# tudoroancea/ihm2

Hardware: AMD Instinct MI355X
Metric: NMPC RTI solves/s (batch), N=40, nx=8 (6-DOF bicycle), fkin6 (higher is better)
Workload: dtype f64

## Files before the change

ihm2_amd/csrc/kernels_qp.hip:

```cpp
#include <cstring>

#include "ihm2mpc_internal.h"
#include "device_steps.hpp"
#include "sqp_body.hpp"
#include "irk_body.hpp"
#include "riccati_mfma.hpp"
#include "sens_body.hpp"
#include "qp_lds.hpp"
#include "qp_catalogue.hpp"
#include "wave_sync.hpp"

using namespace ihm2;

namespace {

#define INF_BOUND 1e20
#ifndef RIC_RING
#define RIC_RING 4
#endif
#ifndef SWEEP_RING
#define SWEEP_RING 4
#endif
#define SWEEP_DL ((SWEEP_RING >= 8) ? 4 : 2)

__device__ __forceinline__ bool fin(double v) { return fabs(v) < INF_BOUND; }
__device__ __forceinline__ int here(int v) { asm volatile("" : "+v"(v)); return v; }

template <typename OP>
__device__ __forceinline__ double wave_reduce(double v, OP op)
{
    v = op(v, dpp_mov<0xB1>(v));
    v = op(v, dpp_mov<0x4E>(v));
    v = op(v, dpp_mov<0x141>(v));
    v = op(v, dpp_mov<0x128>(v));
    int lo = __double2loint(v), hi = __double2hiint(v);
    auto a16 = __builtin_amdgcn_permlane16_swap(lo, lo, false, false);
    auto b16 = __builtin_amdgcn_permlane16_swap(hi, hi, false, false);
    v = op(__hiloint2double(b16[0], a16[0]), __hiloint2double(b16[1], a16[1]));
    lo = __double2loint(v); hi = __double2hiint(v);
    auto a32 = __builtin_amdgcn_permlane32_swap(lo, lo, false, false);
    auto b32 = __builtin_amdgcn_permlane32_swap(hi, hi, false, false);
    return op(__hiloint2double(b32[0], a32[0]), __hiloint2double(b32[1], a32[1]));
}
__device__ __forceinline__ double nanmax(double a, double b) { return (a != a || b != b) ? NAN : fmax(a, b); }
__device__ __forceinline__ double wave_max(double v) { return wave_reduce(v, [](double a, double b) { return fmax(a, b); }); }
__device__ __forceinline__ double wave_min(double v) { return wave_reduce(v, [](double a, double b) { return fmin(a, b); }); }
__device__ __forceinline__ double wave_sum(double v) { return wave_reduce(v, [](double a, double b) { return a + b; }); }
__device__ __forceinline__ double wave_nanmax(double v) { return wave_reduce(v, [](double a, double b) { return nanmax(a, b); }); }

__device__ __forceinline__ double sum8(double v)
{
    v += dpp_mov<0xB1>(v);
    v += dpp_mov<0x4E>(v);
    v += dpp_mov<0x141>(v);
    return v;
}

__device__ __forceinline__ double sum_stride8(double v)
{
    v += dpp_mov<0x128>(v);
    int lo = __double2loint(v), hi = __double2hiint(v);
    auto a16 = __builtin_amdgcn_permlane16_swap(lo, lo, false, false);
    auto b16 = __builtin_amdgcn_permlane16_swap(hi, hi, false, false);
    v = __hiloint2double(b16[0], a16[0]) + __hiloint2double(b16[1], a16[1]);
    lo = __double2loint(v); hi = __double2hiint(v);
    auto a32 = __builtin_amdgcn_permlane32_swap(lo, lo, false, false);
    auto b32 = __builtin_amdgcn_permlane32_swap(hi, hi, false, false);
    return __hiloint2double(b32[0], a32[0]) + __hiloint2double(b32[1], a32[1]);
}

template <int DIR, int D, int DL, bool BUF = true, typename P, typename F>
__device__ __forceinline__ void stream_rows(const double *rows, int N, int e_even, int e_odd, P &&pre, F &&body)
{
    static_assert(D % 2 == 0 && DL % 2 == 0 && D % DL == 0 && 3 * D <= QM_PAD, "the element index alternates with the step parity");
    double r[2][D], x0[DL], x1[DL];
    const __amdgpu_buffer_rsrc_t rsrc = __builtin_amdgcn_make_buffer_rsrc(const_cast<double *>(rows) - (size_t)QM_PAD * 64, 0, (N + 2 * QM_PAD) * 512, 0x00020000);
    const unsigned ve = (unsigned)e_even * 8u, vo = (unsigned)e_odd * 8u;
    typedef unsigned int u2_t __attribute__((ext_vector_type(2)));
    const double *p_even = rows + (size_t)((DIR < 0) ? N - 1 : 0) * 64 + e_even, *p_odd = rows + (size_t)((DIR < 0) ? N - 1 : 0) * 64 + e_odd;
    auto load_row = [&](const int step, const bool odd) -> double {
        if constexpr (BUF) {
            const int row = (DIR < 0) ? N - 1 - step : step;
            const u2_t v = __builtin_amdgcn_raw_buffer_load_b64(rsrc, odd ? vo : ve, (QM_PAD + row) * 512, 0);
            return __hiloint2double((int)v.y, (int)v.x);
        } else
            return (odd ? p_odd : p_even)[(ptrdiff_t)DIR * step * 64];
    };
#pragma unroll
    for (int d = 0; d < D; d++) {
        r[0][d] = load_row(d, (d & 1) != 0);
        __builtin_amdgcn_sched_barrier(0);
        if (d < DL) pre((DIR < 0) ? N - 1 - d : d, (d & 1) != 0, x0[d], x1[d]);
    }
    for (int s0 = 0; s0 < N; s0 += 2 * D) {
#pragma unroll
        for (int h = 0; h < 2; h++) {
#pragma unroll
            for (int d = 0; d < D; d++) {
                const int s = s0 + h * D + d;
                const int k = (DIR < 0) ? N - 1 - s : s;
                const double v = r[h][d], y0 = x0[d % DL], y1 = x1[d % DL];
                r[h ^ 1][d] = load_row(s + D, (d & 1) != 0);
                pre((DIR < 0) ? k - DL : k + DL, (d & 1) != 0, x0[d % DL], x1[d % DL]);
                if (s < N) body(k, v, (d & 1) != 0, y0, y1);
            }
        }
    }
}
template <int DIR, int D, int DL, typename P, typename F>
__device__ __forceinline__ void stream_rows_v1(const double *rows, int N, int e_even, int e_odd, P &&pre, F &&body)
{
    stream_rows<DIR, D, DL, false>(rows, N, e_even, e_odd, pre, body);
}

template <int NSLOT, int NSOFT, int PATH, int UNI, int NW = 1, int LEAN = 1, int NF = 0, int FULL = 0>
__device__ __forceinline__ void qp_wave_body(const QpArgs &a, const int b, double *sm, const bool want_res = true)
{
    static_assert(NF == 0 || NW == 1, "the straight-line factor sweep parks its idle lanes' stores in the tile the block reductions use");
    static_assert(FULL == 0 || (NSOFT == 0 && PATH == 0 && UNI != 0 && NW == 1 && LEAN != 0 && NF > 0 && NSLOT <= 8),
                  "the full slot form is written for the all-hard table of the batch-shared rows, one wave, the lean phases and the compiled-in horizon");
    constexpr int NT = 64 * NW;
    const int tid = threadIdx.x, lane = tid & 63, wv = tid >> 6;
#define BSYNC() do { if (NW == 1) WSYNC(); else __syncthreads(); } while (0)
    const int N = (NF > 0) ? NF : a.N, NS = N + 1;
    constexpr QpLdsClass CLS = qp_lds_class(PATH, UNI != 0);
    constexpr int NCK = CLS.nck;
    const double *Hs0 = a.Hs + (size_t)b * a.hs_bs, *HsT = Hs0 + a.hs_te;
    const double *Gy0 = a.Gy + (size_t)b * a.gy_bs, *GyT = Gy0 + a.gy_te;
    const double *slot_lbb = a.slot_lb + (size_t)b * a.sl_bs, *slot_ubb = a.slot_ub + (size_t)b * a.sl_bs;
    constexpr bool ALAT = PATH == 2;
    constexpr bool HL = CLS.hl, CL = CLS.cl;
    static_assert(qp_factor_inside(qp_lds(40, CLS), 40, NCK) && qp_factor_inside(qp_lds(2, CLS), 2, NCK), "factor stage / block reductions leave their LDS");
    static_assert(qp_sweeps_inside(qp_lds(40, CLS), 40, LEAN != 0, SWEEP_RING, SWEEP_DL) && (LEAN == 0 || qp_sweeps_inside(qp_lds(2, CLS), 2, true, SWEEP_RING, SWEEP_DL)),
                  "the sweeps' unclamped LDS prefetch leaves the block (the earlier form does below N = 4: api.hip refuses those launches)");
    static_assert(NW <= 4, "qp_factor_inside checks the block reductions for four waves");
    static_assert(FULL == 0 || qp_full_zeroes_kept(qp_lds(NF > 0 ? NF : 2, CLS), NF > 0 ? NF : 2), "a store of the factor sweep reaches gam or cf: the full slot form zeroes them once per solve");
#define LEN(id) qp_lds_len(id, N, NS, CLS)
    double *z = sm, *gt = z + LEN(QP_Z), *pi = gt + LEN(QP_GT), *pv = pi + LEN(QP_PI), *rb = pv + LEN(QP_PV), *gam = rb + LEN(QP_RB), *cf = gam + LEN(QP_GAM), *dz = cf + LEN(QP_CF);
    double *kff = dz + LEN(QP_DZ), *Kl = kff + LEN(QP_KFF), *Ginv = Kl + LEN(QP_KL), *Prb = Ginv + LEN(QP_GINV), *tile = Prb + LEN(QP_PRB), *hc = tile + LEN(QP_TILE), *ha = hc + LEN(QP_HC);
    double *Hl = ha + LEN(QP_HA), *CDl = Hl + LEN(QP_HL), *spv = CDl + LEN(QP_CDL);
    int *spc = reinterpret_cast<int *>(spv + 60);
#undef LEN
#define HS(k, i, l) (HL ? Hl[(((k) == N) ? 100 : 0) + (i) * 10 + (l)] : ((k) == N ? HsT : Hs0 + (UNI ? 0 : (k)) * 100)[(i) * 10 + (l)])
#define CDV(k, r, j) (CL ? CDl[(r) * 10 + (j)] : a.CD[((k) * 2 + (r)) * 10 + (j)])

    auto blk_reduce = [&](double v, auto op) -> double {
        v = wave_reduce(v, op);
        if (NW > 1) {
            __syncthreads();
            if (lane == 0) tile[wv] = v;
            __syncthreads();
            v = tile[0];
#pragma unroll
            for (int w = 1; w < NW; w++) v = op(v, tile[w]);
        }
        return v;
    };
    auto blk_max = [&](double v) { return blk_reduce(v, [](double x, double y) { return fmax(x, y); }); };
    auto blk_min = [&](double v) { return blk_reduce(v, [](double x, double y) { return fmin(x, y); }); };
    auto blk_sum = [&](double v) { return blk_reduce(v, [](double x, double y) { return x + y; }); };
    auto blk_nanmax = [&](double v) { return blk_reduce(v, [](double x, double y) { return nanmax(x, y); }); };

    const double *xb = a.x + (size_t)b * NS * 8;
    const double *ub = a.u + (size_t)b * N * 2;
    const double *linb = a.lin + (size_t)b * N * LIN_REC;
    double *gb = a.g + (size_t)b * NS * 10;
    double *rgb = a.rg + (size_t)b * NS * 10;
    double *Pg = a.P + (size_t)b * NS * 64;
    double *Mg = a.M + (size_t)b * N * 64;
    double *pib = a.pi + (size_t)b * NS * 8;
    double *lamb = a.lam + (size_t)b * NS * 28;
    double *slkb = a.slk + (size_t)b * NS * 28;
    double *lamab = ALAT ? a.lam_a + (size_t)b * NS * 2 : nullptr;
    double *slkab = ALAT ? a.slk_a + (size_t)b * NS * 2 : nullptr;
    auto alat_slot = [](int j) -> int { return (j == 3) ? 0 : (j == 4) ? 1 : (j == 6) ? 2 : (j == 7) ? 3 : -1; };

    if (HL) for (int e = tid; e < 200; e += NT) Hl[e] = (e < 100) ? Hs0[e] : HsT[e - 100];
    if (CL && tid < 20) CDl[tid] = a.CD[tid];
    if (UNI) BSYNC();
    bool h_sparse = false;
    if (HL) {
        int cnt = 0;
        if (tid < 20) {
#pragma unroll
            for (int l = 0; l < 10; l++) {
                const double v = Hl[tid * 10 + l];
                if (v != 0.0) { if (cnt < 3) { spv[tid * 3 + cnt] = v; spc[tid * 3 + cnt] = l; } cnt++; }
            }
            for (int q = cnt; q < 3; q++) { spv[tid * 3 + q] = 0.0; spc[tid * 3 + q] = 0; }
        }
        h_sparse = __ballot(cnt > 3) == 0ull;
        if (NW > 1) h_sparse = blk_max((wv == 0 && !h_sparse) ? 1.0 : 0.0) == 0.0;
        BSYNC();
    }
    double sg = 1.0, sb = 1.0, r_stat = 0.0, r_eq = 0.0;
    double w_R = 0.0, w_L = 0.0;
    if (PATH) {
        const int trk = a.track_id[b];
        w_R = a.widths[trk * 2 + 0]; w_L = a.widths[trk * 2 + 1];
        for (int k = tid; k < NS; k += NT) {
            const double psi = xb[k * 8 + 2], sgn = (psi > 0.0) - (psi < 0.0);
            const double dfoot = -0.5 * a.car_L * cos(fabs(psi)) * sgn, dlat = -0.5 * a.car_W * sin(psi);
            hc[k * 2 + 0] = (k >= 1) ? dfoot + dlat : 0.0;
            hc[k * 2 + 1] = (k >= 1) ? -dfoot + dlat : 0.0;
            if (ALAT) {
                double g4[4];
                alat_eval(xb[k * 8 + 3], xb[k * 8 + 4], xb[k * 8 + 6], xb[k * 8 + 7], g4);
#pragma unroll
                for (int q = 0; q < 4; q++) ha[k * 4 + q] = (k >= 1 && k < N) ? g4[q] : 0.0;
            }
        }
        BSYNC();
    }
    for (int e = tid; e < NS * 10; e += NT) {
        const int k = e / 10, j = e % 10;
        double acc = 0.0;
#pragma unroll
        for (int l = 0; l < 8; l++) acc = fma(HS(k, j, l), xb[k * 8 + l], acc);
        if (k < N) {
            acc = fma(HS(k, j, 8), ub[k * 2 + 0], acc);
            acc = fma(HS(k, j, 9), ub[k * 2 + 1], acc);
            const double *yr = a.yref + ((size_t)b * N + k) * 12;
#pragma unroll
            for (int l = 0; l < 12; l++) acc = fma(-Gy0[((UNI ? 0 : k) * 10 + j) * 12 + l], yr[l], acc);
        } else {
            const double *yr = a.yref_e + (size_t)b * 8;
#pragma unroll
            for (int l = 0; l < 8; l++) acc = fma(-GyT[j * 12 + l], yr[l], acc);
        }
        gb[e] = acc;
        const bool counted = !((k == 0 && j < 8) || (k == N && j >= 8));
        if (j < 8 || k < N) sg = fmax(sg, fabs(acc));
        if (!want_res) continue;
        double st = acc;
        if (k < N) {
            const double *rec = linb + (size_t)k * LIN_REC;
#pragma unroll
            for (int l = 0; l < 8; l++) st = fma((j < 8) ? rec[l * 8 + j] : rec[64 + l * 2 + (j - 8)], pib[(k + 1) * 8 + l], st);
        }
        if (j < 8) st -= pib[k * 8 + j];
        st -= lamb[k * 28 + j] - lamb[k * 28 + 14 + j];
        if (k < N) {
            st = fma(-CDV(k, 0, j), lamb[k * 28 + 10] - lamb[k * 28 + 24], st);
            st = fma(-CDV(k, 1, j), lamb[k * 28 + 11] - lamb[k * 28 + 25], st);
        }
        if (PATH && (j == 1 || j == 2)) {
            const double l12 = lamb[k * 28 + 12] - lamb[k * 28 + 26], l13 = lamb[k * 28 + 13] - lamb[k * 28 + 27];
            st -= (j == 1) ? l12 - l13 : hc[k * 2] * l12 + hc[k * 2 + 1] * l13;
        }
        if (ALAT && alat_slot(j) >= 0) st -= ha[k * 4 + alat_slot(j)] * (lamab[k * 2] - lamab[k * 2 + 1]);
        if (counted) r_stat = fmax(r_stat, fabs(st));
    }
    for (int e = tid; e < N * 8; e += NT) {
        const double bl = linb[(size_t)(e / 8) * LIN_REC + 80 + (e % 8)];
        sb = fmax(sb, fabs(bl));
        r_eq = fmax(r_eq, fabs(bl));
    }
    if (tid < 8) {
        const double d = a.x0[(size_t)b * 8 + tid] - xb[tid];
        sb = fmax(sb, fabs(d));
        r_eq = fmax(r_eq, fabs(d));
    }
    sg = blk_max(sg); sb = blk_max(sb);

    int s_kc[NSLOT];
    double s_dl[NSLOT], s_du[NSLOT];
    double lam_l[NSLOT], lam_u[NSLOT], t_l[NSLOT], t_u[NSLOT];
    constexpr int NSO = (NSOFT > 0) ? NSOFT : 1;
    double so_zw[NSO], so_Zw[NSO], so_s[NSO], so_ls[NSO], so_rs[NSO], so_ds[NSO], so_dls[NSO], so_pa[NSO];
#pragma unroll
    for (int r = 0; r < NSO; r++) { so_zw[r] = 0.0; so_Zw[r] = -1.0; so_s[r] = 1.0; so_ls[r] = 0.0; so_rs[r] = 0.0; so_ds[r] = so_dls[r] = so_pa[r] = 0.0; }
#define IS_SOFT(r) ((r) < NSOFT && so_Zw[(r) < NSOFT ? (r) : 0] >= 0.0)
#define ONE_SIDED(r) (NSOFT > 0 && PATH != 2 && (r) < NSOFT)
#define HAS_L(r) (FULL ? true : ONE_SIDED(r) ? true : fin(s_dl[r]))
// ... 158 lines not shown
            }
            __syncthreads();
            mu_acc = 0.0;
            for (int sidx = lane; sidx < a.nslots_can; sidx += 64) mu_acc = __dadd_rn(mu_acc, gam[sidx]);
            __syncthreads();
        }
        if (LEAN == 0) BSYNC();
        for (int rpass = 0; rpass < 2; rpass++) {
            if (exact) {
                for (int e = tid; e < NS * 10; e += NT) {
                    const int k = e / 10, j = e % 10;
                    double acc = gb[e];
                    if (HL && h_sparse) {
                        const int row = ((k == N) ? 10 : 0) + j;
#pragma unroll
                        for (int q = 0; q < 3; q++) acc = fma(spv[row * 3 + q], z[k * 10 + spc[row * 3 + q]], acc);
                    } else {
#pragma unroll
                        for (int l = 0; l < 10; l++) acc = fma(HS(k, j, l), z[k * 10 + l], acc);
                    }
                    if (k < N) {
                        acc = fma(-CDV(k, 0, j), cf[k * NCK + 10], acc);
                        acc = fma(-CDV(k, 1, j), cf[k * NCK + 11], acc);
                    }
                    if (j < 8) acc -= pi[k * 8 + j];
                    acc -= cf[k * NCK + j];
                    if (PATH && (j == 1 || j == 2)) {
                        const double l12 = cf[k * NCK + 12], l13 = cf[k * NCK + 13];
                        acc -= (j == 1) ? l12 - l13 : hc[k * 2] * l12 + hc[k * 2 + 1] * l13;
                    }
                    if (ALAT && alat_slot(j) >= 0) acc -= ha[k * 4 + alat_slot(j)] * cf[k * NCK + 14];
                    gt[e] = acc;
                }
                BSYNC();
                dyn_residual<4, NT>(N, tid, const_cast<double *>(linb), z, pi, gt, rb, LIN_REC);
                BSYNC();
            }
            res_g = 0.0; res_b = 0.0;
            if (exact || LEAN == 0) {
                for (int e = tid; e < NS * 10; e += NT) {
                    const int k = e / 10, j = e % 10;
                    double v = gt[e];
                    if ((k == 0 && j < 8) || (k == N && j >= 8)) { v = 0.0; gt[e] = 0.0; }
                    if (exact) rgb[e] = v;
                    res_g = nanmax(res_g, fabs(v));
                }
                for (int e = tid; e < N * 8; e += NT) res_b = nanmax(res_b, fabs(rb[e]));
            } else { res_g = fol_g; res_b = fol_b; }
            res_g = nanmax(res_g, res_gs);
            res_g = blk_nanmax(res_g); res_b = blk_nanmax(res_b);
            if (rpass == 0) { res_d = blk_nanmax(res_d); res_m = blk_nanmax(res_m); mu = ((NW == 1) ? blk_sum(mu_acc) : wave_sum(mu_acc)) * inv_m; }
            if (!(res_g == res_g) || !(res_b == res_b) || !(res_d == res_d) || !(res_m == res_m)) { qstatus = (it == 0) ? 3 : 4; finished = true; break; }
            const bool conv = res_g <= tol_g && res_b <= tol_b && res_d <= tol_d && res_m <= tol_m;
            if (conv && exact) { qstatus = 0; finished = true; break; }
            if ((conv || it >= a.iter_max) && !exact) {
                exact = true; exact_mode = true;
                if (LEAN != 0) multipliers_to_cf();
                continue;
            }
            break;
        }
        if (finished) break;
        if (it >= a.iter_max) { qstatus = 1; break; }
        BSYNC();
        double alpha = 1.0, alpha_d = 1.0, sigma = 0.0;
        auto slot_coeffs = [&](int pass) {
            if (!FULL) {
                for (int e = tid; e < NS * NCK; e += NT) { cf[e] = 0.0; if (pass == 0) gam[e] = 0.0; }
                BSYNC();
            }
            const double mu_t = fmax(sigma * mu, mu_floor);
#pragma unroll
            for (int r = 0; r < NSLOT; r++) {
                if (NO_SLOT(r)) continue;
                const bool al = HAS_L(r), au = HAS_U(r);
                double c = 0.0;
                if (IS_SOFT(r)) {
                    const int q = r < NSOFT ? r : 0;
                    const double lm = al ? lam_l[r] : lam_u[r], tt = al ? t_l[r] : t_u[r], rdv = al ? rd_l[r] : rd_u[r];
                    const double gm = lm / tt, gs = so_ls[q] / so_s[q], D = so_Zw[q] + gm + gs;
                    double c1, c2, rsv;
                    if (pass == 0) { c1 = (lm * tt + lm * rdv) / tt; c2 = so_ls[q]; rsv = so_rs[q]; SLOT_AT(gam, r) += gm * (so_Zw[q] + gs) / D; }
                    else { c1 = ((al ? pa_l[r] : pa_u[r]) - mu_t) / tt; c2 = (so_pa[q] - mu_t) / so_s[q]; rsv = 0.0; }
                    c = c1 - gm * (rsv + c1 + c2) / D;
                    SLOT_AT(cf, r) += ONE_SIDED(r) ? ROW_SIGN(r, c) : (al ? c : -c);
                    continue;
                }
                if (pass == 0) {
                    const double gl = al ? lam_l[r] / t_l[r] : 0.0, gu = au ? lam_u[r] / t_u[r] : 0.0;
                    if (al) c += fma(gl, rd_l[r], lam_l[r]);
                    if (au) c -= fma(gu, rd_u[r], lam_u[r]);
                    SLOT_ACC(SLOT_AT(gam, r), gl + gu);
                } else {
                    if (al) c += (pa_l[r] - mu_t) / t_l[r];
                    if (au) c -= (pa_u[r] - mu_t) / t_u[r];
                }
                SLOT_ACC(SLOT_AT(cf, r), ROW_SIGN(r, c));
            }
            BSYNC();
        };
        auto add_coeffs = [&]() {
            for (int e = tid; e < NS * 10; e += NT) {
                const int k = e / 10, j = e % 10;
                double acc = gt[e] + cf[k * NCK + j];
                if (k < N) {
                    acc = fma(CDV(k, 0, j), cf[k * NCK + 10], acc);
                    acc = fma(CDV(k, 1, j), cf[k * NCK + 11], acc);
                }
                if (PATH && (j == 1 || j == 2)) {
                    const double c12 = cf[k * NCK + 12], c13 = cf[k * NCK + 13];
                    acc += (j == 1) ? c12 - c13 : hc[k * 2] * c12 + hc[k * 2 + 1] * c13;
                }
                if (ALAT && alat_slot(j) >= 0) acc += ha[k * 4 + alat_slot(j)] * cf[k * NCK + 14];
                gt[e] = acc;
            }
            BSYNC();

        };
        slot_coeffs(0);
        add_coeffs();
        __builtin_amdgcn_s_waitcnt(0x0F70);
        if (wv == 0) {
            RicLds L;
            const QpRic o = qp_lds_ric(N, NS, NCK);
            L.gt = o.gt; L.pv = o.pv; L.gam = o.gam; L.dz = o.dz; L.kff = o.kff; L.Kl = o.Kl;
            L.Ginv = o.Ginv; L.hv = o.Prb; L.tile = o.tile; L.hc = o.hc; L.ha = o.ha;
            if constexpr (NF != 0)
                riccati_sweep_mfma<NCK, PATH != 0, UNI != 0, RIC_RING, ALAT, true, (NF > 0) ? NF : 0>(N, lane, linb, Hs0, HsT, a.CD, L, Pg, Mg, LIN_REC, false, false);
            else
            riccati_sweep_mfma<NCK, PATH != 0, UNI != 0, RIC_RING, ALAT>(N, lane, linb, Hs0, HsT, a.CD, L, Pg, Mg, LIN_REC, a.m_act == 0, a.symmetrize != 0);
            if (lane < 8) dz[lane] = 0.0;
        }
        BSYNC();
        for (int pass = 0; pass < 2; pass++) {
            const double mu_t = fmax(sigma * mu, mu_floor);
            if (pass == 1) slot_coeffs(1);
            if (pass == 1) {
            add_coeffs();
            for (int e = tid; e < NS * 8; e += NT) {
                const int k = e >> 3, j = e & 7;
                double v = gt[k * 10 + j];
                if (k < N) v -= Kl[k * 16 + j] * gt[k * 10 + 8] + Kl[k * 16 + 8 + j] * gt[k * 10 + 9];
                pv[e] = v;
            }
            BSYNC();
            if constexpr (LEAN != 0) {
            if (wv == 0) {
                const int g = lane >> 3, w = lane & 7;
                double pw = pv[N * 8 + w], pg = 0.0;
                const int se2 = (w == 0) ? 16 : 0, so2 = (g == 0) ? 16 : 0;
                const double *be = (w == 0) ? pv + (N - 1) * 8 + g : dz, *bo = (g == 0) ? pv + (N - 2) * 8 + w : dz;
                const double *qe = Prb + (N - 1) * 8 + w, *qo = Prb + (N - 2) * 8 + g;
                double *oe = pv + (N - 1) * 8 + g, *oo = pv + (N - 2) * 8 + w;
                stream_rows<-1, SWEEP_RING, SWEEP_DL>(Mg, N, RIC_IDX(w, g), RIC_IDX(g, w),
                    [&](int k, bool odd, double &prb, double &base) {
                        if (odd) { prb = *qo; qo -= 16; base = *bo; bo -= so2; } else { prb = *qe; qe -= 16; base = *be; be -= se2; }
                    },
                    [&](int k, double m, bool odd, double prb, double base) {
                        if (!odd) {
                            pg = sum8(fma(m, pw, fma(m, prb, base)));
                            *oe = pg; oe -= 16;
                        } else {
                            pw = sum_stride8(fma(m, pg, fma(m, prb, base)));
                            *oo = pw; oo -= 16;
                        }
                    });
            }
            } else {
            if (wv == 0) {
                const int g = lane >> 3, w = lane & 7;
                double pw = pv[N * 8 + w], pg = 0.0;
                stream_rows_v1<-1, QP_V1_RING, QP_V1_DL>(Mg, N, RIC_IDX(w, g), RIC_IDX(g, w),
                    [&](int k, bool odd, double &prb, double &base) { prb = Prb[k * 8 + (odd ? g : w)]; base = pv[k * 8 + (odd ? w : g)]; },
                    [&](int k, double m, bool odd, double prb, double base) {
                        if (!odd) {
                            const double off = fma(m, prb, (w == 0) ? base : 0.0);
                            pg = sum8(fma(m, pw, off));
                            if (w == 0) pv[k * 8 + g] = pg;
                        } else {
                            const double off = fma(m, prb, (g == 0) ? base : 0.0);
                            pw = sum_stride8(fma(m, pg, off));
                            if (g == 0) pv[k * 8 + w] = pw;
                        }
                    });
            }
            }
            BSYNC();
            for (int k = tid; k < N; k += NT) {
                const double *rec = linb + (size_t)k * LIN_REC;
                double g0 = gt[k * 10 + 8], g1 = gt[k * 10 + 9];
                double Bk[16];
#pragma unroll
                for (int l = 0; l < 16; l++) Bk[l] = rec[64 + l];
#pragma unroll
                for (int l = 0; l < 8; l++) {
                    const double h = Prb[k * 8 + l] + pv[(k + 1) * 8 + l];
                    g0 = fma(Bk[l * 2 + 0], h, g0);
                    g1 = fma(Bk[l * 2 + 1], h, g1);
                }
                const double kf0 = Ginv[k * 8 + 0] * g0 + Ginv[k * 8 + 1] * g1;
                const double kf1 = Ginv[k * 8 + 1] * g0 + Ginv[k * 8 + 2] * g1;
                kff[k * 4 + 0] = kf0;
                kff[k * 4 + 1] = kf1;
#pragma unroll
                for (int i = 0; i < 8; i++) dz[(k + 1) * 10 + i] = rb[k * 8 + i] - Bk[i * 2] * kf0 - Bk[i * 2 + 1] * kf1;
            }
            if (tid < 8) dz[tid] = 0.0;
            BSYNC();
            }

            if constexpr (LEAN != 0) {
            if (wv == 0) {
                const int g = lane >> 3, w = lane & 7;
                double dxw = dz[w], dxg = 0.0;
                const int se2 = (w == 0) ? 20 : 0, so2 = (g == 0) ? 20 : 0;
                const double *ce = (w == 0) ? dz + 10 + g : dz, *co = (g == 0) ? dz + 20 + w : dz;
                stream_rows<+1, SWEEP_RING, SWEEP_DL>(Mg, N, RIC_IDX(g, w), RIC_IDX(w, g),
                    [&](int k, bool odd, double &c, double &unused) {
                        if (odd) { c = *co; co += so2; } else { c = *ce; ce += se2; }
                        unused = 0.0;
                    },
                    [&](int k, double m, bool odd, double c, double) {
                        if (!odd) {
                            dxg = sum8(fma(m, dxw, c));
                            dz[(k + 1) * 10 + g] = dxg;
                        } else {
                            dxw = sum_stride8(fma(m, dxg, c));
                            dz[(k + 1) * 10 + w] = dxw;
                        }
                    });
            }
            } else {
            if (wv == 0) {
                const int g = lane >> 3, w = lane & 7;
                double dxw = dz[w], dxg = 0.0;
                stream_rows_v1<+1, QP_V1_RING, QP_V1_DL>(Mg, N, RIC_IDX(g, w), RIC_IDX(w, g),
                    [&](int k, bool odd, double &c, double &unused) { c = dz[(k + 1) * 10 + (odd ? w : g)]; unused = 0.0; },
                    [&](int k, double m, bool odd, double c, double) {
                        if (!odd) {
                            dxg = sum8(fma(m, dxw, (w == 0) ? c : 0.0));
                            if (w == 0) dz[(k + 1) * 10 + g] = dxg;
                        } else {
                            dxw = sum_stride8(fma(m, dxg, (g == 0) ? c : 0.0));
                            if (g == 0) dz[(k + 1) * 10 + w] = dxw;
                        }
                    });
            }
            }
            BSYNC();
            const bool want_dpi = (pass == 1) || (a.m_act == 0);
            for (int e = tid; e < NS * 2; e += NT) {
                const int k = e >> 1, aa = e & 1;
                double acc = 0.0;
                if (k < N) {
                    acc = -kff[k * 4 + aa];
#pragma unroll
                    for (int l = 0; l < 8; l++) acc = fma(-Kl[k * 16 + aa * 8 + l], dz[k * 10 + l], acc);
                }
                dz[k * 10 + 8 + aa] = acc;
            }
            if (want_dpi) {
                const int n = NS * 8;
                for (int base = 0; base < n; base += 3 * NT) {
                    double2 pr[3][4];
#pragma unroll
                    for (int q = 0; q < 3; q++) {
                        const int e = min(base + NT * q + tid, n - 1), k = e >> 3, i = e & 7;
#pragma unroll
                        for (int l = 0; l < 4; l++) pr[q][l] = *reinterpret_cast<const double2 *>(Pg + (size_t)k * 64 + RIC_IDX(l, i));
                    }
#pragma unroll
                    for (int q = 0; q < 3; q++) {
                        const int e = base + NT * q + tid, ec = min(e, n - 1), k = ec >> 3;
                        double acc = pv[ec];
#pragma unroll
                        for (int l = 0; l < 4; l++) { acc = fma(pr[q][l].x, dz[k * 10 + l], acc); acc = fma(pr[q][l].y, dz[k * 10 + l + 4], acc); }
                        if (e < n) pv[e] = acc;
                    }
                }
            }
            BSYNC();

            double amax = 1.0, amax_d = 1.0, mu_aff = 0.0, rmax = 1.0, rmax_d = 1.0;
#pragma unroll
            for (int r = 0; r < NSLOT; r++) {
                dlam_l[r] = dlam_u[r] = dt_l[r] = dt_u[r] = 0.0;
                if (NO_SLOT(r)) continue;
                const double drz = ROW_DOT(r, dz);
                if (IS_SOFT(r)) {
                    const int q = r < NSOFT ? r : 0;
                    const bool al = HAS_L(r);
                    const double lm = al ? lam_l[r] : lam_u[r], tt = al ? t_l[r] : t_u[r], rdv = al ? rd_l[r] : rd_u[r];
                    const double y = al ? drz : -drz;
                    const double gm = lm / tt, gs = so_ls[q] / so_s[q], D = so_Zw[q] + gm + gs;
                    const double rm1 = (pass == 0) ? lm * tt : lm * tt + (al ? pa_l[r] : pa_u[r]) - mu_t;
                    const double rm2 = (pass == 0) ? so_ls[q] * so_s[q] : so_ls[q] * so_s[q] + so_pa[q] - mu_t;
                    const double c1 = (rm1 + lm * rdv) / tt, c2 = rm2 / so_s[q];
                    const double dsv = -(so_rs[q] + c1 + c2) / D - gm / D * y;
                    const double dlsv = -(rm2 + so_ls[q] * dsv) / so_s[q];
                    const double dtv = y + dsv + rdv;
                    const double dlv = -(rm1 + lm * dtv) / tt;
                    so_ds[q] = dsv; so_dls[q] = dlsv;
                    if (al) { dt_l[r] = dtv; dlam_l[r] = dlv; } else { dt_u[r] = dtv; dlam_u[r] = dlv; }
                    if (dsv < 0.0) amax = fmin(amax, -so_s[q] / dsv);
                    if (dlsv < 0.0) amax_d = fmin(amax_d, -so_ls[q] / dlsv);
                    if (dtv < 0.0) amax = fmin(amax, -tt / dtv);
                    if (dlv < 0.0) amax_d = fmin(amax_d, -lm / dlv);
                    continue;
                }
                if (HAS_L(r)) {
                    const double rm = (pass == 0) ? lam_l[r] * t_l[r] : lam_l[r] * t_l[r] + pa_l[r] - mu_t;
                    dt_l[r] = drz + rd_l[r];
                    if (NSOFT == 0) {
                        const double it = 1.0 / t_l[r];
                        dlam_l[r] = -(rm + lam_l[r] * dt_l[r]) * it;
                        rmax = fmax(rmax, -dt_l[r] * it);
                        rmax_d = fmax(rmax_d, -dlam_l[r] / lam_l[r]);
                    } else {
                        dlam_l[r] = -(rm + lam_l[r] * dt_l[r]) / t_l[r];
                        if (dt_l[r] < 0.0) amax = fmin(amax, -t_l[r] / dt_l[r]);
                        if (dlam_l[r] < 0.0) amax_d = fmin(amax_d, -lam_l[r] / dlam_l[r]);
                    }
                }
                if (HAS_U(r)) {
                    const double rm = (pass == 0) ? lam_u[r] * t_u[r] : lam_u[r] * t_u[r] + pa_u[r] - mu_t;
                    dt_u[r] = -drz + rd_u[r];
                    if (NSOFT == 0) {
                        const double it = 1.0 / t_u[r];
                        dlam_u[r] = -(rm + lam_u[r] * dt_u[r]) * it;
                        rmax = fmax(rmax, -dt_u[r] * it);
                        rmax_d = fmax(rmax_d, -dlam_u[r] / lam_u[r]);
                    } else {
                        dlam_u[r] = -(rm + lam_u[r] * dt_u[r]) / t_u[r];
                        if (dt_u[r] < 0.0) amax = fmin(amax, -t_u[r] / dt_u[r]);
                        if (dlam_u[r] < 0.0) amax_d = fmin(amax_d, -lam_u[r] / dlam_u[r]);
                    }
                }
            }
            if (NSOFT == 0) { amax = fmin(amax, 1.0 / rmax); amax_d = fmin(amax_d, 1.0 / rmax_d); }
            amax = blk_min(amax); amax_d = blk_min(amax_d);
            if (pass == 0) {
                if (a.m_act == 0) { alpha = alpha_d = 1.0; break; }
#pragma unroll
                for (int r = 0; r < NSLOT; r++) {
                    pa_l[r] = dlam_l[r] * dt_l[r]; pa_u[r] = dlam_u[r] * dt_u[r];
                    if (NO_SLOT(r)) continue;
                    mu_aff = __dadd_rn(mu_aff, __dadd_rn(HAS_L(r) ? __dmul_rn(fma(amax_d, dlam_l[r], lam_l[r]), fma(amax, dt_l[r], t_l[r])) : 0.0,
                                                         HAS_U(r) ? __dmul_rn(fma(amax_d, dlam_u[r], lam_u[r]), fma(amax, dt_u[r], t_u[r])) : 0.0));
                    if (IS_SOFT(r)) {
                        const int q = r < NSOFT ? r : 0;
                        so_pa[q] = so_dls[q] * so_ds[q];
                        mu_aff += (so_ls[q] + amax_d * so_dls[q]) * (so_s[q] + amax * so_ds[q]);
                    }
                }
                if constexpr (NW > 1) {
#pragma unroll
                    for (int r = 0; r < NSLOT; r++) {
                        const int sidx = tid + NT * r;
                        if (sidx >= a.nslots_can) continue;
                        const bool on = s_kc[r] >= 0;
                        gam[sidx] = __dadd_rn((on && fin(s_dl[r])) ? __dmul_rn(fma(amax_d, dlam_l[r], lam_l[r]), fma(amax, dt_l[r], t_l[r])) : 0.0,
                                              (on && fin(s_du[r])) ? __dmul_rn(fma(amax_d, dlam_u[r], lam_u[r]), fma(amax, dt_u[r], t_u[r])) : 0.0);
                    }
                    __syncthreads();
                    mu_aff = 0.0;
                    for (int sidx = lane; sidx < a.nslots_can; sidx += 64) mu_aff = __dadd_rn(mu_aff, gam[sidx]);
                    __syncthreads();
                    mu_aff = wave_sum(mu_aff) * inv_m;
                } else
                mu_aff = blk_sum(mu_aff) * inv_m;
// ... 342 lines not shown
```

ihm2_amd/csrc/riccati_mfma.hpp:

```cpp
#pragma once
#ifdef RIC_STAMPS
__device__ long long ric_dbg[8];
#define RIC_STAMP_DECL long long ric_T[8] = {0, 0, 0, 0, 0, 0, 0, 0}, ric_tp = __builtin_readcyclecounter(); int ric_cur = 7;
#define RIC_STAMP(i) do { const long long t_now = __builtin_readcyclecounter(); ric_T[ric_cur] += t_now - ric_tp; ric_tp = t_now; ric_cur = (i); } while (0)
#define RIC_STAMP_OUT do { if (threadIdx.x == 0 && blockIdx.x == 0) for (int q = 0; q < 8; q++) ric_dbg[q] = ric_T[q]; } while (0)
#else
#define RIC_STAMP_DECL
#define RIC_STAMP(i)
#define RIC_STAMP_OUT
#endif

#include <hip/hip_runtime.h>

#include "qp_lds.hpp"
#include "wave_sync.hpp"

namespace ihm2 {

typedef double d4_t __attribute__((ext_vector_type(4)));
#define IHM2_MFMA_F64(a, b, c) __builtin_amdgcn_mfma_f64_16x16x4f64((a), (b), (c), 0, 0, 0)

template <int CTRL>
__device__ __forceinline__ double dpp_mov(double v)
{
    int lo = __double2loint(v), hi = __double2hiint(v);
    lo = __builtin_amdgcn_mov_dpp(lo, CTRL, 0xF, 0xF, false);
    hi = __builtin_amdgcn_mov_dpp(hi, CTRL, 0xF, 0xF, false);
    return __hiloint2double(hi, lo);
}
__device__ __forceinline__ double readlane_f64(double v, int lane)
{
    return __hiloint2double(__builtin_amdgcn_readlane(__double2hiint(v), lane), __builtin_amdgcn_readlane(__double2loint(v), lane));
}

#define RIC_IDX(row, col) (((((row) & 3) * 8 + (col)) << 1) + ((row) >> 2))
#define RIC_REC_RB 88

struct RicLds {
    int gam;
    int hc;
    int ha;
    int gt;
    int pv;
    int hv;
    int Kl;
    int Ginv;
    int kff;
    int dz;
    int tile;
};

template <int NB, int NT = 64>
__device__ __forceinline__ void dyn_residual(const int N, const int lane, double *linb, const double *z, const double *pi, double *gt, double *rb,
                                             const int lin_rec)
{
    const int n1 = N * 8;
    for (int base = 0; base < n1; base += NT * NB) {
        double2 Ar[NB][4], Br[NB];
        double br[NB];
#pragma unroll
        for (int q = 0; q < NB; q++) {
            const int e = min(base + NT * q + lane, n1 - 1), k = e >> 3, o = e & 7;
            const double *rec = linb + (size_t)k * lin_rec;
            const double2 *row = reinterpret_cast<const double2 *>(rec + o * 8);
#pragma unroll
            for (int l = 0; l < 4; l++) Ar[q][l] = row[l];
            Br[q] = *reinterpret_cast<const double2 *>(rec + 64 + o * 2);
            br[q] = rec[80 + o];
        }
#pragma unroll
        for (int q = 0; q < NB; q++) {
            const int e = base + NT * q + lane, ec = min(e, n1 - 1), k = ec >> 3, o = ec & 7;
            double acc = br[q] - z[(k + 1) * 10 + o];
#pragma unroll
            for (int l = 0; l < 4; l++) { acc = fma(Ar[q][l].x, z[k * 10 + 2 * l], acc); acc = fma(Ar[q][l].y, z[k * 10 + 2 * l + 1], acc); }
            acc = fma(Br[q].x, z[k * 10 + 8], acc);
            acc = fma(Br[q].y, z[k * 10 + 9], acc);
            if (e < n1) {
                rb[e] = acc;
                linb[(size_t)k * lin_rec + RIC_REC_RB + o] = acc;
            }
        }
    }
    const int n2 = N * 10;
    for (int base = 0; base < n2; base += NT * NB) {
        double cr[NB][8];
#pragma unroll
        for (int q = 0; q < NB; q++) {
            const int e = min(base + NT * q + lane, n2 - 1), k = e / 10, jz = e - k * 10;
            const double *rec = linb + (size_t)k * lin_rec;
            const double *col = (jz < 8) ? rec + jz : rec + 64 + (jz - 8);
            const int cs = (jz < 8) ? 8 : 2;
#pragma unroll
            for (int l = 0; l < 8; l++) cr[q][l] = col[l * cs];
        }
#pragma unroll
        for (int q = 0; q < NB; q++) {
            const int e = base + NT * q + lane, ec = min(e, n2 - 1), k = ec / 10;
            double acc = gt[ec];
#pragma unroll
            for (int l = 0; l < 8; l++) acc = fma(cr[q][l], pi[(k + 1) * 8 + l], acc);
            if (e < n2) gt[e] = acc;
        }
    }
}

template <int NCK, bool PATH, bool UNI, int D, bool ALAT = false, bool PLAIN = false, int NF = 0>
__device__ __forceinline__ void riccati_sweep_mfma(const int N_rt, const int lane, const double *__restrict__ linb, const double *__restrict__ Hs,
                                                   const double *__restrict__ HsT,
                                                   const double *__restrict__ CD, const RicLds L, double *__restrict__ Pg, double *__restrict__ Mg,
                                                   const int lin_rec, const bool store_p, const bool symmetrize)
{
    static_assert(!PLAIN || (UNI && !PATH && !ALAT), "the straight-line stage is written for the batch-shared all-hard tables");
    static_assert(PLAIN || NF == 0, "a compile-time horizon comes with the straight-line stage");
    const int N = (NF > 0) ? NF : N_rt;
    const int g = lane >> 4, j = lane & 15;
    const int col = (j < 10) ? j : (j == 12) ? 9 : (j == 13) ? 8 : -1;
    const int row[4] = {g, g + 4, (g < 2) ? 8 + g : -1, (g == 0) ? 9 : (g == 1) ? 8 : -1};
    const double m10 = (j == 10) ? 1.0 : 0.0;
    extern __shared__ double ric_sm[];
#define sm ric_sm

    unsigned off[2], offB;
#pragma unroll
    for (int c = 0; c < 2; c++) {
        const int rr = 4 * c + g;
        off[c] = (j < 8) ? rr * 8 + j : (col >= 0) ? 64 + rr * 2 + (col - 8) : RIC_REC_RB + rr;
    }
    offB = (j >= 8) ? 64 + (j - 8) * 2 + (g & 1) : 0;
    double hconst[4], cc0[4], cc1[4], dsel[4];
    int va[4], vstride[4];
#pragma unroll
    for (int r = 0; r < 4; r++) {
        const bool ok = row[r] >= 0 && col >= 0, gr = row[r] >= 0 && j == 10;
        hconst[r] = (UNI && ok) ? Hs[row[r] * 10 + col] : 0.0;
        cc0[r] = (UNI && ok) ? CD[row[r]] * CD[col] : 0.0;
        cc1[r] = (UNI && ok) ? CD[10 + row[r]] * CD[10 + col] : 0.0;
        dsel[r] = ((ok && row[r] == col) || gr) ? 1.0 : 0.0;
        vstride[r] = (j == 10) ? 10 : NCK;
        va[r] = ((j == 10) ? L.gt : L.gam) + ((r == 3) ? ((row[3] >= 0) ? row[3] : 0) : g) + (N - 1) * vstride[r];
    }
    int a_g10 = L.gam + (N - 1) * NCK + 10;
    const double p11 = (PATH && row[0] == 1 && col == 1) ? 1.0 : 0.0, p22 = (PATH && row[0] == 2 && col == 2) ? 1.0 : 0.0;
    const double p12 = (PATH && ((row[0] == 1 && col == 2) || (row[0] == 2 && col == 1))) ? 1.0 : 0.0;
    auto a_slot = [](int c) -> int { return (c == 3) ? 0 : (c == 4) ? 1 : (c == 6) ? 2 : (c == 7) ? 3 : -1; };
    const int as_c = ALAT ? a_slot(col) : -1, as_r0 = ALAT ? a_slot(row[0]) : -1, as_r1 = ALAT ? a_slot(row[1]) : -1;
    const double am0 = (as_c >= 0 && as_r0 >= 0) ? 1.0 : 0.0, am1 = (as_c >= 0 && as_r1 >= 0) ? 1.0 : 0.0;
    const int ao_c = L.ha + max(as_c, 0), ao_r0 = L.ha + max(as_r0, 0), ao_r1 = L.ha + max(as_r1, 0);
    const double selA0 = (g == 0) ? 1.0 : 0.0, selA2 = (g == 1) ? 1.0 : 0.0, selB = (g < 2) ? -1.0 : 0.0;

    const int a_tw = L.tile + g * QP_TILE_ROW + j, a_tr = L.tile + (j & 7) * QP_TILE_ROW + g;
    const double wS = (j < 8) ? 0.5 : 1.0, wT = (j < 8) ? 0.5 : 0.0;

    d4_t Pd;
    {
        const double g12 = PATH ? sm[L.gam + N * NCK + 12] : 0.0, g13 = PATH ? sm[L.gam + N * NCK + 13] : 0.0;
        const double a0 = PATH ? sm[L.hc + N * 2] : 0.0, a1 = PATH ? sm[L.hc + N * 2 + 1] : 0.0;
#pragma unroll
        for (int r = 0; r < 2; r++) {
            double v = 0.0;
            if (j < 8) {
                v = HsT[row[r] * 10 + j];
                if (row[r] == j) v += sm[L.gam + N * NCK + j];
            } else if (j == 10) v = sm[L.gt + N * 10 + row[r]];
            if (PATH && r == 0) v += p11 * (g12 + g13) + p12 * (g12 * a0 - g13 * a1) + p22 * (g12 * a0 * a0 + g13 * a1 * a1);
            Pd[r] = v;
            if (j < 8) Pg[(size_t)N * 64 + RIC_IDX(row[r], j)] = v;
            if (j == 10) sm[L.pv + N * 8 + row[r]] = v;
        }
        Pd[2] = Pd[3] = 0.0;
    }

    double r0[D], r1[D], rB[D];
    const int rec_bytes = lin_rec * 8;
    const __amdgpu_buffer_rsrc_t rsrc = __builtin_amdgcn_make_buffer_rsrc(const_cast<double *>(linb), 0, PLAIN ? N * rec_bytes : 0, 0x00020000);
    const unsigned vo0 = off[0] * 8u, vo1 = off[1] * 8u, voB = offB * 8u;
    typedef unsigned int ric_u2_t __attribute__((ext_vector_type(2)));
    auto rec_load = [&](const unsigned voff, const int soff) -> double {
        const ric_u2_t v = __builtin_amdgcn_raw_buffer_load_b64(rsrc, voff, soff, 0);
        return __hiloint2double((int)v.y, (int)v.x);
    };
#pragma unroll
    for (int d = 0; d < D; d++) {
        if constexpr (PLAIN) {
            const int so = max(N - 1 - d, 0) * rec_bytes;
            r0[d] = rec_load(vo0, so); r1[d] = rec_load(vo1, so); rB[d] = rec_load(voB, so);
        } else {
            const double *rec = linb + (size_t)max(N - 1 - d, 0) * lin_rec;
            r0[d] = rec[off[0]]; r1[d] = rec[off[1]]; rB[d] = rec[offB];
        }
    }
    int rs = (N - 1 - D) * rec_bytes;
    unsigned gofs = (unsigned)((N - 1) * 64 + RIC_IDX(g, j)) * 8u;
    const bool own10 = j == 10, ownK = j < 8 && g < 2;
    const int dead = L.tile + lane;
    int a_hv = own10 ? L.hv + (N - 1) * 8 + g : dead, a_dz = own10 ? L.dz + N * 10 + g : dead, a_gi = own10 ? L.Ginv + (N - 1) * 8 + 2 * g : dead;
    int a_kf = own10 ? L.kff + (N - 1) * 4 + g : ownK ? L.Kl + (N - 1) * 16 + g * 8 + j : dead;
    const int st8 = own10 ? 8 : 0, st10 = own10 ? 10 : 0, stk = own10 ? 4 : ownK ? 16 : 0;
    d4_t Hc;
    double val[4], g10, g11, pg12 = 0.0, pg13 = 0.0, pa0 = 0.0, pa1 = 0.0, pg14 = 0.0, pac = 0.0, par0 = 0.0, par1 = 0.0;
    auto prepare_load = [&](const int k) {
        val[0] = sm[va[0]]; val[1] = sm[va[0] + 4]; val[2] = sm[va[0] + 8]; val[3] = sm[va[3]];
        g10 = sm[a_g10]; g11 = sm[a_g10 + 1];
        if (PATH) { pg12 = sm[a_g10 + 2]; pg13 = sm[a_g10 + 3]; pa0 = sm[L.hc + k * 2]; pa1 = sm[L.hc + k * 2 + 1]; }
        if (ALAT) { pg14 = sm[a_g10 + 4]; pac = sm[ao_c + k * 4]; par0 = sm[ao_r0 + k * 4]; par1 = sm[ao_r1 + k * 4]; }
        a_g10 -= NCK;
        va[0] -= vstride[0]; va[3] -= vstride[3];
    };
    auto prepare_compute = [&](const int k) {
        double hk[4], c0k[4], c1k[4];
#pragma unroll
        for (int r = 0; r < 4; r++) { hk[r] = hconst[r]; c0k[r] = cc0[r]; c1k[r] = cc1[r]; }
        if (!UNI) {
#pragma unroll
            for (int r = 0; r < 4; r++) {
                const bool ok = row[r] >= 0 && col >= 0;
                hk[r] = ok ? Hs[(k * 10 + row[r]) * 10 + col] : 0.0;
                c0k[r] = ok ? CD[(k * 2 + 0) * 10 + row[r]] * CD[(k * 2 + 0) * 10 + col] : 0.0;
                c1k[r] = ok ? CD[(k * 2 + 1) * 10 + row[r]] * CD[(k * 2 + 1) * 10 + col] : 0.0;
            }
        }
#pragma unroll
        for (int r = 0; r < 4; r++) Hc[r] = fma(g11, c1k[r], fma(g10, c0k[r], fma(dsel[r], val[r], hk[r])));
        if (PATH) Hc[0] += p11 * (pg12 + pg13) + p12 * (pg12 * pa0 - pg13 * pa1) + p22 * (pg12 * pa0 * pa0 + pg13 * pa1 * pa1);
        if (ALAT) { Hc[0] += am0 * pg14 * par0 * pac; Hc[1] += am1 * pg14 * par1 * pac; }
    };
    prepare_load(N - 1);
    prepare_compute(N - 1);
    RIC_STAMP_DECL
    for (int s0 = 0; s0 < N; s0 += D) {
#pragma unroll
        for (int d = 0; d < D; d++) {
            const int s = s0 + d;
            const int k = N - 1 - s;
            if ((NF > 0 && NF % D == 0) || s < N) {
                RIC_STAMP(0);
                const double B0 = r0[d], B1 = r1[d], Bmk = rB[d];
                const d4_t Hk = Hc;
                const double q0 = m10 * Pd[0], q1 = m10 * Pd[1];
                d4_t W = {q0, q1, 0.0, 0.0};
                W = IHM2_MFMA_F64(Pd[0], B0, W);
                W = IHM2_MFMA_F64(Pd[1], B1, W);
                RIC_STAMP(1);
                d4_t G = Hk;
                G = IHM2_MFMA_F64(B0, W[0], G);
                G = IHM2_MFMA_F64(B1, W[1], G);
                RIC_STAMP(2);
                const double g00 = readlane_f64(G[2], 8), g01 = readlane_f64(G[2], 9), g11u = readlane_f64(G[2], 25);
                const double det = g00 * g11u - g01 * g01;
                double idet = __builtin_amdgcn_rcp(det);
                const double cAa = selA0 * g11u + selA2 * g00, cBa = selB * g01;
                const double ta = cAa * G[2] + cBa * G[3];
                idet = fma(fma(-det, idet, 1.0), idet, idet);
                idet = fma(fma(-det, idet, 1.0), idet, idet);
                const double Kf = ta * idet;
                RIC_STAMP(3);
                const double Sa = (j < 8) ? G[2] : Bmk;
                d4_t S = {G[0], G[1], B0, B1};
                S = IHM2_MFMA_F64(Sa, -Kf, S);
                RIC_STAMP(4);
                if constexpr (PLAIN) {
                    {
                        const int so = max(rs, 0);
                        r0[d] = rec_load(vo0, so); r1[d] = rec_load(vo1, so); rB[d] = rec_load(voB, so);
                        rs -= rec_bytes;
                    }
                    prepare_load(k - 1);
                    RIC_STAMP(5);
                    sm[a_hv] = W[0] - q0; sm[a_hv + 4] = W[1] - q1;
                    sm[a_dz] = S[2]; sm[a_dz + 4] = S[3];
                    sm[a_gi] = cAa * idet; sm[a_gi + 1] = cBa * idet;
                    sm[a_kf] = Kf;
                    a_hv -= st8; a_gi -= st8; a_dz -= st10; a_kf -= stk;
                    Pd[0] = S[0]; Pd[1] = S[1];
                    prepare_compute(k - 1);
                    if (j < 8) {
                        double2 mm, pp;
                        mm.x = S[2]; mm.y = S[3];
                        pp.x = S[0]; pp.y = S[1];
                        *(double2 *)((char *)Mg + gofs) = mm;
                        *(double2 *)((char *)Pg + gofs) = pp;
                    }
                    gofs -= 512u;
                } else {
                if (symmetrize) { sm[a_tw] = S[0]; sm[a_tw + 4 * QP_TILE_ROW] = S[1]; }
                {
                    const double *rec = linb + (size_t)max(k - D, 0) * lin_rec;
                    r0[d] = rec[off[0]]; r1[d] = rec[off[1]]; rB[d] = rec[offB];
                }
                if (k > 0) prepare_load(k - 1);
                RIC_STAMP(5);
#ifndef RIC_SKIP_A
                if (j < 8) {
                    double2 mm;
                    mm.x = S[2]; mm.y = S[3];
                    *(double2 *)(Mg + (size_t)k * 64 + RIC_IDX(g, j)) = mm;
                    if (g < 2) sm[L.Kl + k * 16 + g * 8 + j] = Kf;
                }
#endif
#ifndef RIC_SKIP_B
                if (j == 10) {
                    sm[L.hv + k * 8 + g] = W[0] - q0; sm[L.hv + k * 8 + 4 + g] = W[1] - q1;
                    if (store_p) { sm[L.pv + k * 8 + g] = S[0]; sm[L.pv + k * 8 + 4 + g] = S[1]; }
                    sm[L.dz + (k + 1) * 10 + g] = S[2]; sm[L.dz + (k + 1) * 10 + 4 + g] = S[3];
                    sm[L.Ginv + k * 8 + 2 * g] = cAa * idet; sm[L.Ginv + k * 8 + 2 * g + 1] = cBa * idet;
                    sm[L.kff + k * 4 + g] = Kf;
                }
#endif
                WSYNC();
                if (symmetrize) {
                    const double T0 = sm[a_tr], T1 = sm[a_tr + 4];
                    Pd[0] = fma(wT, T0, wS * S[0]);
                    Pd[1] = fma(wT, T1, wS * S[1]);
                } else { Pd[0] = S[0]; Pd[1] = S[1]; }
                if (k > 0) prepare_compute(k - 1);
#ifndef RIC_SKIP_A
                if (j < 8) {
                    double2 pp;
                    pp.x = Pd[0]; pp.y = Pd[1];
                    *(double2 *)(Pg + (size_t)k * 64 + RIC_IDX(g, j)) = pp;
                }
#endif
                }
                RIC_STAMP(6);
            }
        }
    }
    RIC_STAMP_OUT;
#undef sm
}

}
```

Before: 1.290 million.

## Interleave consecutive stages' M rows so sweeps fetch two stages per 128-bit load

For compiled-in horizons, the Riccati factor pass now writes the M matrices in a paired layout: each lane's element for an even and the following odd stage sit side by side, with the odd stage stored transposed. The lean backward and forward sweeps then pull both stages with a single 128-bit buffer load per lane instead of two 64-bit loads. This halves the number of load instructions in the latency-bound sweeps. In exchange, the odd-stage writes in the factor pass become two scalar stores instead of one double2 store, and the indexing assumes an even horizon.

```diff
diff --git a/ihm2_amd/csrc/kernels_qp.hip b/ihm2_amd/csrc/kernels_qp.hip
--- a/ihm2_amd/csrc/kernels_qp.hip
+++ b/ihm2_amd/csrc/kernels_qp.hip
@@ -7,6 +7,7 @@
 #include "riccati_mfma.hpp"
 #include "sens_body.hpp"
 #include "qp_lds.hpp"
+#include "qp_mrows.hpp"
 #include "qp_catalogue.hpp"
 #include "wave_sync.hpp"
 
@@ -69,10 +70,50 @@
     return __hiloint2double(b32[0], a32[0]) + __hiloint2double(b32[1], a32[1]);
 }
 
-template <int DIR, int D, int DL, bool BUF = true, typename P, typename F>
+template <int DIR, int D, int DL, bool BUF = true, bool PAIR = false, typename P, typename F>
 __device__ __forceinline__ void stream_rows(const double *rows, int N, int e_even, int e_odd, P &&pre, F &&body)
 {
     static_assert(D % 2 == 0 && DL % 2 == 0 && D % DL == 0 && 3 * D <= QM_PAD, "the element index alternates with the step parity");
+    if constexpr (PAIR) {
+        static_assert(BUF, "the paired rows come through buffer loads");
+        typedef unsigned int u4_t __attribute__((ext_vector_type(4)));
+        u4_t r2[D];
+        double x0[DL], x1[DL];
+        const __amdgpu_buffer_rsrc_t rsrc = __builtin_amdgcn_make_buffer_rsrc(const_cast<double *>(rows) - (size_t)QM_PAD * 64, 0, (N + 2 * QM_PAD) * QM_STAGE_BYTES, 0x00020000);
+        const unsigned vl = (unsigned)qm_pair_slot(2, 0, (int)threadIdx.x & 63);
+        auto load_pair = [&](const int pstep) -> u4_t {
+            const int prow = (DIR < 0) ? (N >> 1) - 1 - pstep : pstep;
+            return __builtin_amdgcn_raw_buffer_load_b128(rsrc, vl, QM_PAD * QM_STAGE_BYTES + prow * QM_PAIR_BYTES, 0);
+        };
+        auto half = [&](const u4_t v, const bool odd) -> double {
+            const bool second = (DIR < 0) ? !odd : odd;
+            return second ? __hiloint2double((int)v.w, (int)v.z) : __hiloint2double((int)v.y, (int)v.x);
+        };
+#pragma unroll
+        for (int p = 0; p < D; p++) {
+            r2[p] = load_pair(p);
+            __builtin_amdgcn_sched_barrier(0);
+            if (p < DL) pre((DIR < 0) ? N - 1 - p : p, (p & 1) != 0, x0[p], x1[p]);
+        }
+        for (int s0 = 0; s0 < N; s0 += 2 * D) {
+#pragma unroll
+            for (int p = 0; p < D; p++) {
+#pragma unroll
+                for (int t = 0; t < 2; t++) {
+                    const int s = s0 + 2 * p + t;
+                    const int k = (DIR < 0) ? N - 1 - s : s;
+                    const double v = half(r2[p], t != 0), y0 = x0[(2 * p + t) % DL], y1 = x1[(2 * p + t) % DL];
+                    pre((DIR < 0) ? k - DL : k + DL, t != 0, x0[(2 * p + t) % DL], x1[(2 * p + t) % DL]);
+                    if (s < N) body(k, v, t != 0, y0, y1);
+                    if (t == 1) {
+                        r2[p] = load_pair((s0 >> 1) + p + D);
+                        __builtin_amdgcn_sched_barrier(0);
+                    }
+                }
+            }
+        }
+        return;
+    }
     double r[2][D], x0[DL], x1[DL];
     const __amdgpu_buffer_rsrc_t rsrc = __builtin_amdgcn_make_buffer_rsrc(const_cast<double *>(rows) - (size_t)QM_PAD * 64, 0, (N + 2 * QM_PAD) * 512, 0x00020000);
     const unsigned ve = (unsigned)e_even * 8u, vo = (unsigned)e_odd * 8u;
@@ -120,6 +161,9 @@
     static_assert(FULL == 0 || (NSOFT == 0 && PATH == 0 && UNI != 0 && NW == 1 && LEAN != 0 && NF > 0 && NSLOT <= 8),
                   "the full slot form is written for the all-hard table of the batch-shared rows, one wave, the lean phases and the compiled-in horizon");
     constexpr int NT = 64 * NW;
+    constexpr bool PAIRM = NF > 0;
+    static_assert(!PAIRM || (NF % 4 == 0 && LEAN != 0 && NW == 1 && qm_pair_inside(NF > 0 ? NF : 2, SWEEP_RING, QM_PAD)),
+                  "the paired rows: an even horizon in whole factor passes, the lean sweeps, and their unclamped prefetch inside q_M's padding");
     const int tid = threadIdx.x, lane = tid & 63, wv = tid >> 6;
 #define BSYNC() do { if (NW == 1) WSYNC(); else __syncthreads(); } while (0)
     const int N = (NF > 0) ? NF : a.N, NS = N + 1;
@@ -584,7 +628,7 @@
                 const double *be = (w == 0) ? pv + (N - 1) * 8 + g : dz, *bo = (g == 0) ? pv + (N - 2) * 8 + w : dz;
                 const double *qe = Prb + (N - 1) * 8 + w, *qo = Prb + (N - 2) * 8 + g;
                 double *oe = pv + (N - 1) * 8 + g, *oo = pv + (N - 2) * 8 + w;
-                stream_rows<-1, SWEEP_RING, SWEEP_DL>(Mg, N, RIC_IDX(w, g), RIC_IDX(g, w),
+                stream_rows<-1, SWEEP_RING, SWEEP_DL, true, PAIRM>(Mg, N, RIC_IDX(w, g), RIC_IDX(g, w),
                     [&](int k, bool odd, double &prb, double &base) {
                         if (odd) { prb = *qo; qo -= 16; base = *bo; bo -= so2; } else { prb = *qe; qe -= 16; base = *be; be -= se2; }
                     },
@@ -647,7 +691,7 @@
                 double dxw = dz[w], dxg = 0.0;
                 const int se2 = (w == 0) ? 20 : 0, so2 = (g == 0) ? 20 : 0;
                 const double *ce = (w == 0) ? dz + 10 + g : dz, *co = (g == 0) ? dz + 20 + w : dz;
-                stream_rows<+1, SWEEP_RING, SWEEP_DL>(Mg, N, RIC_IDX(g, w), RIC_IDX(w, g),
+                stream_rows<+1, SWEEP_RING, SWEEP_DL, true, PAIRM>(Mg, N, RIC_IDX(g, w), RIC_IDX(w, g),
                     [&](int k, bool odd, double &c, double &unused) {
                         if (odd) { c = *co; co += so2; } else { c = *ce; ce += se2; }
                         unused = 0.0;
diff --git a/ihm2_amd/csrc/qp_mrows.hpp b/ihm2_amd/csrc/qp_mrows.hpp
--- /dev/null
+++ b/ihm2_amd/csrc/qp_mrows.hpp
@@ -0,0 +1,49 @@
+#pragma once
+
+#ifdef __HIPCC__
+#define QP_MROWS_FN __host__ __device__ constexpr
+#else
+#define QP_MROWS_FN constexpr
+#endif
+
+namespace ihm2 {
+
+constexpr int QM_STAGE_BYTES = 512, QM_PAIR_BYTES = 2 * QM_STAGE_BYTES;
+
+QP_MROWS_FN int qm_stage_byte(int k, int row, int col) { return k * QM_STAGE_BYTES + (((((row & 3) * 8 + col) << 1) + (row >> 2)) << 3); }
+
+QP_MROWS_FN bool qm_pair_horizon(int N) { return N > 0 && N % 2 == 0; }
+QP_MROWS_FN int qm_pair_write(int N, int k, int row, int col)
+{
+    if (!qm_pair_horizon(N) || k < 0 || k >= N) return -1;
+    return ((k >> 1) * 64 + ((k & 1) ? col * 8 + row : row * 8 + col)) * 16 + (k & 1) * 8;
+}
+QP_MROWS_FN int qm_pair_slot(int N, int k, int lane) { return qm_pair_horizon(N) ? ((k >> 1) * 64 + lane) * 16 : -1; }
+QP_MROWS_FN int qm_pair_read(int N, int k, int lane, bool backward)
+{
+    if (!qm_pair_horizon(N) || k < 0 || k >= N) return -1;
+    const int step = backward ? N - 1 - k : k;
+    const int half = backward ? 1 - (step & 1) : (step & 1);
+    return qm_pair_slot(N, k, lane) + half * 8;
+}
+QP_MROWS_FN int qm_sweep_row(int lane, bool backward, bool odd_step) { return (backward != odd_step) ? (lane & 7) : (lane >> 3); }
+QP_MROWS_FN int qm_sweep_col(int lane, bool backward, bool odd_step) { return (backward != odd_step) ? (lane >> 3) : (lane & 7); }
+
+struct QmReach { int lo, hi; };
+QP_MROWS_FN int qm_pair_rows_fetched(int N, int ring) { return ((N + 2 * ring - 1) / (2 * ring) + 1) * ring; }
+QP_MROWS_FN QmReach qm_pair_reach(int N, int ring)
+{
+    return {(N / 2 - qm_pair_rows_fetched(N, ring)) * QM_PAIR_BYTES, qm_pair_rows_fetched(N, ring) * QM_PAIR_BYTES};
+}
+QP_MROWS_FN bool qm_pair_inside(int N, int ring, int pad_rows)
+{
+    const QmReach r = qm_pair_reach(N, ring);
+    return qm_pair_horizon(N) && r.lo >= -pad_rows * QM_STAGE_BYTES && r.hi <= (N + pad_rows) * QM_STAGE_BYTES;
+}
+
+static_assert(qm_pair_write(40, 38, 3, 5) == qm_stage_byte(38, 3, 5) && qm_pair_write(40, 0, 0, 7) == qm_stage_byte(0, 0, 7), "even stages: same byte for rows 0..3");
+QP_MROWS_FN int qm_pair_odd_delta(int N, int g, int j) { return qm_pair_write(N, 1, g, j) - qm_stage_byte(1, g, j); }
+QP_MROWS_FN int qm_pair_row4_step(int N, bool odd) { return qm_pair_write(N, odd ? 1 : 0, 4, 0) - qm_pair_write(N, odd ? 1 : 0, 0, 0); }
+static_assert(qm_pair_row4_step(40, false) == 512 && qm_pair_row4_step(40, true) == 64, "rows g and g + 4 of a column: 32 lanes or 4 lanes apart");
+
+}
diff --git a/ihm2_amd/csrc/riccati_mfma.hpp b/ihm2_amd/csrc/riccati_mfma.hpp
--- a/ihm2_amd/csrc/riccati_mfma.hpp
+++ b/ihm2_amd/csrc/riccati_mfma.hpp
@@ -13,6 +13,7 @@
 #include <hip/hip_runtime.h>
 
 #include "qp_lds.hpp"
+#include "qp_mrows.hpp"
 #include "wave_sync.hpp"
 
 namespace ihm2 {
@@ -192,6 +193,8 @@
     }
     int rs = (N - 1 - D) * rec_bytes;
     unsigned gofs = (unsigned)((N - 1) * 64 + RIC_IDX(g, j)) * 8u;
+    static_assert(NF <= 0 || (NF % D == 0 && D % 2 == 0 && qm_pair_horizon(NF)), "the stage's parity is a constant of the straight-line pass");
+    const unsigned mdel = (NF > 0) ? (unsigned)qm_pair_odd_delta(NF > 0 ? NF : 2, g, j & 7) : 0u;
     const bool own10 = j == 10, ownK = j < 8 && g < 2;
     const int dead = L.tile + lane;
     int a_hv = own10 ? L.hv + (N - 1) * 8 + g : dead, a_dz = own10 ? L.dz + N * 10 + g : dead, a_gi = own10 ? L.Ginv + (N - 1) * 8 + 2 * g : dead;
@@ -278,6 +281,12 @@
                         double2 mm, pp;
                         mm.x = S[2]; mm.y = S[3];
                         pp.x = S[0]; pp.y = S[1];
+                        if constexpr (NF > 0) {
+                            const bool odd_k = ((NF - 1 - d) & 1) != 0;
+                            char *const mp = (char *)Mg + (odd_k ? gofs + mdel : gofs);
+                            *(double *)mp = mm.x;
+                            *(double *)(mp + qm_pair_row4_step(NF, odd_k)) = mm.y;
+                        } else
                         *(double2 *)((char *)Mg + gofs) = mm;
                         *(double2 *)((char *)Pg + gofs) = pp;
                     }
```

Measured after the change: 1.305 million (median of 6 runs). 1.01x the previous value.
